# lancedb/lance

Measured on NVIDIA H100. Metric: ivf_pq_index_build_mvec_per_s, higher is better.
Workload: dtype f32

## Files before the change

### lance_b200/csrc/kmeans.cu

```cuda
#include <cooperative_groups.h>

#include <algorithm>
#include <cmath>
#include <limits>
#include <condition_variable>
#include <deque>
#include <functional>
#include <map>
#include <memory>
#include <mutex>
#include <queue>
#include <thread>
#include <unordered_map>

#include "../../include/lance_b200.h"

#include "assign.cuh"
#include "comm.cuh"
#include "common.cuh"
#include "exact.cuh"
#include "kmeans.cuh"
#include "tc_assign.cuh"
#include "tc_pq.cuh"

// ... 1051 lines not shown
  DevBuf<float> rn2;
  const bool pq_tc = small && ldx == B * ds && tc_pq_supported(n, ldx, B, ds, K, metric, x);
  TcPqPrepArgs pq_prep;
  bool pq_prepared = false;
  if (pq_tc) {
    rn2.alloc(n * B);
    tc_pq_residual_norms(x, nullptr, nullptr, n, B, nullptr, rn2.p);
    pq_prep = tc_pq_prep_args(B, ldx, &pqws);
  }
  sync_stream();
  const PollWords& words = PollWords::reset(B);
  auto iteration = [&]() {
    if (!small) {
      assign_f32_ex(x, n, ds, centroids, K, metric, bias.p, ids.p, dists.p, valid.p, nullptr, active_d.p, tcws);
    } else if (pq_tc) {
      tc_pq_assign(x, rn2.p, n, ldx, B, centroids, nullptr, nullptr, ids.p, dists.p, valid.p,
                   active_d.p, &pqws, pq_prepared);
      pq_prepared = true;
    } else {
      small_d_assign_f32(x, n, ldx, B, ds, centroids, K, metric, nullptr, nullptr, nullptr, nullptr,
                         ids.p, dists.p, valid.p, active_d.p);
    }
    ms.run(ids.p, valid.p, n, K, B, active_d.p);
    const int warp_update = (ds % 8 == 0 && ldx % 4 == 0 && (reinterpret_cast<uintptr_t>(x) & 15) == 0) ? 1 : 0;
    const unsigned ub = warp_update ? cdiv(BK * (uint64_t)(ds / 8), 4) : cdiv(BK * ds, 128);
    const unsigned sb = cdiv((uint64_t)BK * 32, 128);
    LB2_LAUNCH("kmeans_update_stats", update_stats_kernel, ub + sb, 128, 0, ub, x, ldx, ds, K, B, n,
               ms.members.p, ms.offsets.p, dist ? sums_p : centroids, dists.p, losses.p, radius.p,
               last_row.p, active_d.p, dist ? 0 : 1, warp_update, hints.p);
    if (dist) {
      LB2_LAUNCH("kmeans_pack_partials", pack_partials_kernel, cdiv(BK, 256), 256, 0, blob.p, xl, BK, ms.counts.p,
// ... 373 lines not shown
```

### lance_b200/csrc/tc_assign.cu

```cuda
#include <cuda_bf16.h>
#include <cuda_fp16.h>

#include "assign.cuh"
#include "common.cuh"
#include "exact.cuh"
#include "tc_assign.cuh"
#include "tc_common.cuh"

namespace lb2 {

namespace tc {

struct SmemLayout {
  uint32_t b_off, a_off, cnh_off, bar_off, total;
};
__host__ __device__ inline SmemLayout smem_layout(int nkc, int stages) {
  SmemLayout L;
  L.b_off = 0;
  L.a_off = nkc * B_CHUNK_BYTES;
  L.cnh_off = L.a_off + stages * A_STAGE_BYTES;
  L.bar_off = L.cnh_off + TN * 4;
  L.total = L.bar_off + (2 * MAX_STAGES + 1) * 8;
  return L;
}

__device__ __forceinline__ uint32_t verdict(float m1, float m2, float m3, float tau) {
  if (m1 - m2 > tau) return 0;
  if (m1 - m3 > tau) return 1;
  return 2;
}

__global__ void __launch_bounds__(NUM_THREADS, 1)
tc_filter_kernel(const __grid_constant__ CUtensorMap map_x, const __grid_constant__ CUtensorMap map_c,
                 uint64_t n, int nkc, int stages, const float* __restrict__ cnh_g,
                 const float* __restrict__ row_norm2, const float* __restrict__ cn2_g,
                 uint32_t* __restrict__ res, const uint8_t* __restrict__ active, float tau_scale) {
  if (active && !active[0]) return;
  extern __shared__ uint8_t smem_raw[];
  uint8_t* smem = smem_align1024(smem_raw);
  const SmemLayout L = smem_layout(nkc, stages);
  float* cnh = reinterpret_cast<float*>(smem + L.cnh_off);
  uint64_t* bars = reinterpret_cast<uint64_t*>(smem + L.bar_off);
  const uint32_t sb = smem_u32(smem);
  auto full_bar = [&](int s) { return smem_u32(&bars[s]); };
  auto empty_bar = [&](int s) { return smem_u32(&bars[MAX_STAGES + s]); };
  const uint32_t b_full = smem_u32(&bars[2 * MAX_STAGES]);

  const int warp = threadIdx.x >> 5, lane = threadIdx.x & 31;
  const uint64_t num_tiles = (n + TM - 1) / TM;

// ... 27 lines not shown
      for_units_producer(num_tiles, 1, [&](uint64_t tile, int) {
        for (int kc = 0; kc < nkc; ++kc) {
          mbar_wait_relaxed(empty_bar(s), ph ^ 1);
          mbar_expect_tx(full_bar(s), A_STAGE_BYTES);
          tma_load_2d(sb + L.a_off + s * A_STAGE_BYTES, &map_x, full_bar(s), kc * KC, (int)(tile * TM));
          if (++s == stages) { s = 0; ph ^= 1; }
        }
      });
    }
  } else {
    setmaxnreg_inc<CONSUMER_REGS>();
    const int w = (threadIdx.x >> 7) - 1;
    const float cmax2 = s_cmax2;
    float acc[128];
    mbar_wait(b_full, 0);
    for_units_consumer(num_tiles, 1, nkc, w, [&](uint64_t tile, int, uint64_t k, auto pass_turn) {
      mma_unit<0>(acc, nkc,
          [&](int kc, uint32_t& a_addr, uint32_t& b_addr) {
            const uint64_t kk = k + (uint64_t)kc;
            const int s = (int)(kk % (uint64_t)stages);
            mbar_wait(full_bar(s), (uint32_t)((kk / (uint64_t)stages) & 1));
            a_addr = sb + L.a_off + s * A_STAGE_BYTES;
            b_addr = sb + L.b_off + kc * B_CHUNK_BYTES;
            return s;
          },
          [&](int s) {
            __syncwarp();
            if (lane == 0) mbar_arrive(empty_bar(s));
          });
      pass_turn();
      float m[3];
      top3_frag(acc, cnh, m);
      if ((lane & 3) < 2) {
        const uint64_t row = tile * TM + frag_row(lane & 1);
        if (row < n) {
          const uint32_t flag = verdict(m[0], m[1], m[2], tau_scale * (row_norm2[row] + cmax2));
          res[row] = (__float_as_uint(m[0]) & 0xFFu) | ((__float_as_uint(m[1]) & 0xFFu) << 12) | (flag << 30);
        }
      }
    });
  }
}

constexpr int GEN_STAGES = 5;
constexpr int GEN_STAGE_BYTES = A_STAGE_BYTES + B_CHUNK_BYTES;

struct GenLayout {
  uint32_t stage_off, bar_off, total;
};
__host__ __device__ inline GenLayout gen_layout() {
  GenLayout L;
// ... 173 lines not shown
  for (int off = 16; off >= 1; off >>= 1) n2 += __shfl_xor_sync(0xffffffffu, n2, off);
  if (lane == 0) {
    cnh[k] = k < K ? -0.5f * (n2 + (bias ? bias[k] : 0.0f)) : -3.0e38f;
    cn2[k] = (k < K && n2 == n2) ? n2 : 0.0f;
  }
}

__global__ void row_norm_kernel(const float* __restrict__ x, uint64_t n, int d, float* __restrict__ out) {
  const uint64_t hw = ((uint64_t)blockIdx.x * blockDim.x + threadIdx.x) >> 4;
  const int l = threadIdx.x & 15;
  if (hw >= n) return;
  const float* v = x + hw * d;
  float s = 0.0f;
  for (int e = l * 4; e < d; e += 64) {
    const float4 f = *reinterpret_cast<const float4*>(v + e);
    s += f.x * f.x + f.y * f.y + f.z * f.z + f.w * f.w;
  }
  const unsigned mask = 0xffffu << (16 * ((threadIdx.x >> 4) & 1));
#pragma unroll
  for (int off = 8; off >= 1; off >>= 1) s += __shfl_xor_sync(mask, s, off, 16);
  if (l == 0) out[hw] = s;
}

__global__ void __launch_bounds__(256)
rerank_kernel(const float* __restrict__ x, uint64_t n, int d, const float* __restrict__ cent,
              const float* __restrict__ bias, const uint32_t* __restrict__ res,
              const uint32_t* __restrict__ res_hi, int need_dist,
              uint32_t* __restrict__ part, float* __restrict__ dist, uint8_t* __restrict__ valid,
              uint32_t* __restrict__ fb_rows, uint32_t* __restrict__ fb_count,
              const uint8_t* __restrict__ active, const uint32_t* __restrict__ src_list,
              const uint32_t* __restrict__ src_count, uint32_t src_cap, const float* __restrict__ val_in,
// ... 377 lines not shown
                   uint32_t* part, float* dist, uint8_t* valid, const uint8_t* active,
                   TcWorkspace& ws, const void* x16, int x16_dtype) {
  using namespace tc;
  const bool resident = tc_resident_shape(d, K);
  const int ntiles = (K + TN - 1) / TN, Kp = ntiles * TN;
  int stages = MAX_STAGES;
  size_t smem = gen_layout().total + 1024;
  if (resident) {
    SmemLayout L = smem_layout(d / KC, stages);
    while (stages > 2 && L.total + 1024 > ctx().smem_optin) L = smem_layout(d / KC, --stages);
    smem = L.total + 1024;
  }
  if (smem > ctx().smem_optin) fail(LB2_UNSUPPORTED, "tc_assign: shared memory");
  if (ws.cpad.n < (size_t)Kp * d) ws.cpad.alloc((size_t)Kp * d);
  if (ws.cnh.n < (size_t)2 * Kp + 1) ws.cnh.alloc((size_t)2 * Kp + 1);
  if (ws.row_norm2.n < n || ws.norm_src != x || ws.norm_n != n) {
    if (ws.row_norm2.n < n) ws.row_norm2.alloc(n);
    LB2_LAUNCH("tc_row_norms", row_norm_kernel, cdiv(n * 16, 256), 256, 0, x, n, d, ws.row_norm2.p);
    ws.norm_src = x;
    ws.norm_n = n;
  }
  const uint64_t res_n = resident ? n : 2 * n;
  if (ws.res.n < res_n) ws.res.alloc(res_n);
  if (ws.fb_rows.n < n) ws.fb_rows.alloc(n);
  if (ws.fb_count.n < 4) ws.fb_count.alloc(4);
  float* cnh = ws.cnh.p;
  float* cn2 = ws.cnh.p + Kp;
  float* cmax2 = ws.cnh.p + 2 * (size_t)Kp;
  if (resident) {
    const int Kp64 = (K + 63) / 64 * 64;
    if (ws.cT.n < (size_t)d * Kp64) ws.cT.alloc((size_t)d * Kp64);
    LB2_LAUNCH("tc_prep_centroids", prep_centroids_kernel, TN / 8, 256, 0, cent, K, d, bias, ws.cpad.p, cnh, cn2,
               ws.cT.p, Kp64, ws.fb_count.p);
// ... 16 lines not shown
  const unsigned grid = (unsigned)std::min<uint64_t>(tiles, (uint64_t)ctx().num_sms);
  const char* filter = resident ? "tc_filter" : opk ? "tc_filter_general16" : "tc_filter_general";
  if (opk) {
    if (ws.top1_val.n < n) ws.top1_val.alloc(n);
    const CUtensorMap map_x = make_map_2d_16(x16, opk == 2, n, d, TM);
    const CUtensorMap map_c = make_map_2d_16(ws.cpad16.p, opk == 2, Kp, d, TN);
    launch_general_dyn(opk, 0, grid, smem, map_x, map_c, n, d / (2 * KC), ntiles, cnh, ws.row_norm2.p, cmax2, ws.res.p,
                       ws.res.p + n, active, tau16_scale(d), nullptr, 0u, ws.top1_val.p, nullptr, nullptr, nullptr,
                       filter);
  } else {
    const CUtensorMap map_x = make_map_2d(x, n, d, TM);
    const CUtensorMap map_c = make_map_2d(ws.cpad.p, Kp, d, TN);
    if (resident) {
      set_smem(tc_filter_kernel, smem);
      LB2_LAUNCH(filter, tc_filter_kernel, grid, NUM_THREADS, smem, map_x, map_c, n, d / KC, stages, cnh,
                 ws.row_norm2.p, cn2, ws.res.p, active, TAU_TF32);
    } else {
      launch_general_dyn(0, 0, grid, smem, map_x, map_c, n, d / KC, ntiles, cnh, ws.row_norm2.p, cmax2, ws.res.p,
                         ws.res.p + n, active, TAU_TF32, nullptr, 0u, nullptr, nullptr, nullptr, nullptr, filter);
    }
  }
  LB2_LAUNCH("tc_rerank", rerank_kernel, cdiv(n * 16, 256), 256, 0, x, n, d, cent, bias, ws.res.p,
             (const uint32_t*)(resident ? nullptr : ws.res.p + n), dist != nullptr ? 1 : 0, part, dist, valid,
             ws.fb_rows.p, ws.fb_count.p, active, (const uint32_t*)nullptr, (const uint32_t*)nullptr, 0u,
             (const float*)nullptr, (float*)nullptr, (uint32_t*)nullptr, (uint32_t*)nullptr);
  const bool refined = tc_refine_and_fallback(x, n, d, cent, K, Kp, bias, ws.cpad.p, cnh, cmax2, part, dist, valid,
                                              active, ws, resident, opk, x16);
  if (getenv("LB2_TC_STATS") && *getenv("LB2_TC_STATS")) {
    std::vector<uint32_t> h(n);
    uint32_t c[3];
    d2h(h.data(), ws.res.p, n);
// ... 14 lines not shown
```

### lance_b200/csrc/tc_common.cuh

```cuda
#pragma once
#include <cuda.h>
#include <cudaTypedefs.h>
#include <stdint.h>
#include <stdio.h>

#include "common.cuh"

namespace lb2 {
namespace tc {

constexpr int TM = 64;
constexpr int TN = 256;
constexpr int KC = 32;
constexpr int A_STAGE_BYTES = TM * 128;
constexpr int B_CHUNK_BYTES = TN * 128;
constexpr int MAX_STAGES = 6;
constexpr int NUM_THREADS = 384;
constexpr int PRODUCER_REGS = 40, CONSUMER_REGS = 232;

__device__ __forceinline__ uint32_t smem_u32(const void* p) {
  return static_cast<uint32_t>(__cvta_generic_to_shared(p));
}
__device__ __forceinline__ void mbar_init(uint32_t bar, uint32_t count) {
  asm volatile("mbarrier.init.shared::cta.b64 [%0], %1;" ::"r"(bar), "r"(count));
// ... 86 lines not shown
      : "+f"(d[0]), "+f"(d[1]), "+f"(d[2]), "+f"(d[3]), "+f"(d[4]), "+f"(d[5]), "+f"(d[6]), "+f"(d[7]), "+f"(d[8]), "+f"(d[9]), "+f"(d[10]), "+f"(d[11]), "+f"(d[12]), "+f"(d[13]), "+f"(d[14]), "+f"(d[15]), "+f"(d[16]), "+f"(d[17]), "+f"(d[18]), "+f"(d[19]), "+f"(d[20]), "+f"(d[21]), "+f"(d[22]), "+f"(d[23]), "+f"(d[24]), "+f"(d[25]), "+f"(d[26]), "+f"(d[27]), "+f"(d[28]), "+f"(d[29]), "+f"(d[30]), "+f"(d[31]), "+f"(d[32]), "+f"(d[33]), "+f"(d[34]), "+f"(d[35]), "+f"(d[36]), "+f"(d[37]), "+f"(d[38]), "+f"(d[39]), "+f"(d[40]), "+f"(d[41]), "+f"(d[42]), "+f"(d[43]), "+f"(d[44]), "+f"(d[45]), "+f"(d[46]), "+f"(d[47]), "+f"(d[48]), "+f"(d[49]), "+f"(d[50]), "+f"(d[51]), "+f"(d[52]), "+f"(d[53]), "+f"(d[54]), "+f"(d[55]), "+f"(d[56]), "+f"(d[57]), "+f"(d[58]), "+f"(d[59]), "+f"(d[60]), "+f"(d[61]), "+f"(d[62]), "+f"(d[63])
      : "l"(a_desc), "l"(b_desc), "r"(scale_d));
}
__device__ __forceinline__ void wgmma_fence() { asm volatile("wgmma.fence.sync.aligned;" ::: "memory"); }
__device__ __forceinline__ void wgmma_commit() { asm volatile("wgmma.commit_group.sync.aligned;" ::: "memory"); }
template <int N>
__device__ __forceinline__ void wgmma_wait() { asm volatile("wgmma.wait_group.sync.aligned %0;" ::"n"(N) : "memory"); }
__device__ __forceinline__ void wgmma_wait_all() { wgmma_wait<0>(); }
template <int N = 128>
__device__ __forceinline__ void acc_fence(float* d) {
#pragma unroll
  for (int i = 0; i < N; ++i) asm volatile("" : "+f"(d[i])::"memory");
}
__device__ __forceinline__ uint8_t* smem_align1024(uint8_t* raw) {
  return raw + ((1024u - (smem_u32(raw) & 1023u)) & 1023u);
}
template <int OPK>
__device__ __forceinline__ void wgmma_op(float* d, uint64_t a_desc, uint64_t b_desc, uint32_t scale_d) {
  if (OPK == 0) wgmma_tf32(d, a_desc, b_desc, scale_d);
  else if (OPK == 1) wgmma_f16(d, a_desc, b_desc, scale_d);
  else wgmma_bf16(d, a_desc, b_desc, scale_d);
}
template <int OPK, class Stage, class Release>
__device__ __forceinline__ void mma_unit(float* d, int nkc, Stage&& stage, Release&& release) {
  acc_fence(d);
  int prev = -1;
  for (int kc = 0; kc < nkc; ++kc) {
    uint32_t a_addr, b_addr;
    const int s = stage(kc, a_addr, b_addr);
    __syncwarp();
// ... 182 lines not shown
```

### lance_b200/csrc/tc_pq.cu

```cuda
#include "assign.cuh"
#include "common.cuh"
#include "exact.cuh"
#include "tc_common.cuh"
#include "tc_pq.cuh"

namespace lb2 {
namespace tcpq {

using namespace tc;

constexpr int DS = 8;
constexpr int MAX_M_RESIDENT = 16;
constexpr int MAX_M = 256;
constexpr int CNH_CHUNK_BYTES = 4 * TN * 4;
constexpr int STREAM_STAGE_BYTES = A_STAGE_BYTES + B_CHUNK_BYTES + CNH_CHUNK_BYTES;

template <bool STREAM>
struct Pipe {
  static constexpr int CONSUMERS = STREAM ? 2 : 4;
  static constexpr int STAGES = STREAM ? 4 : 8;
  static constexpr int ACC_SETS = STREAM ? 2 : 1;
  static constexpr int THREADS = 128 * (1 + CONSUMERS);
  static constexpr int PRODUCER_REGS = STREAM ? 40 : 24;
  static constexpr int CONSUMER_REGS = STREAM ? 232 : 112;
  static_assert(STAGES % CONSUMERS == 0, "stages are dealt to the consumer warpgroups in turns");
  static_assert(128 * (PRODUCER_REGS + CONSUMERS * CONSUMER_REGS) <= THREADS * ((65536 / THREADS) & ~7),
                "register file");
};

struct Layout {
  uint32_t b_off, a_off, cnh_off, bar_off, cbm_off, misc_off, total;
  uint32_t stage_bytes;
};
__host__ __device__ inline Layout layout(int nkc, int M, bool stream) {
  Layout L;
  if (stream) {
    L.b_off = A_STAGE_BYTES;
    L.a_off = 0;
    L.cnh_off = A_STAGE_BYTES + B_CHUNK_BYTES;
    L.stage_bytes = STREAM_STAGE_BYTES;
    L.bar_off = Pipe<true>::STAGES * STREAM_STAGE_BYTES;
  } else {
    L.b_off = 0;
    L.a_off = nkc * B_CHUNK_BYTES;
    L.cnh_off = L.a_off + Pipe<false>::STAGES * A_STAGE_BYTES;
    L.stage_bytes = A_STAGE_BYTES;
    L.bar_off = L.cnh_off + M * TN * 4;
  }
  static_assert((2 * Pipe<false>::STAGES + 1) * 8 <= 256 && (2 * Pipe<true>::STAGES + 1) * 8 <= 256, "barriers");
  L.cbm_off = L.bar_off + 256;
  L.misc_off = L.cbm_off + MAX_M * 4;
  L.total = L.misc_off + MAX_M;
  return L;
}

__device__ __forceinline__ void bulk_load_1d(uint32_t dst, const void* src, uint32_t bytes, uint32_t bar) {
  asm volatile("cp.async.bulk.shared::cluster.global.mbarrier::complete_tx::bytes [%0], [%1], %2, [%3];"
               ::"r"(dst), "l"(src), "r"(bytes), "r"(bar)
               : "memory");
}

__device__ __forceinline__ const float4* swz(const uint8_t* tile, int r, int u) {
  return reinterpret_cast<const float4*>(tile + (r >> 3) * 1024 + (r & 7) * 128 + ((u ^ (r & 7)) << 4));
}

template <bool TRAIN, bool STREAM>
__global__ void __launch_bounds__(Pipe<STREAM>::THREADS, 1)
tc_pq_kernel(const __grid_constant__ CUtensorMap map_r, const __grid_constant__ CUtensorMap map_b,
             uint64_t n, int M, const float* __restrict__ cnh_g, const float* __restrict__ cbmax2,
             const float* __restrict__ rn2, const uint8_t* __restrict__ row_valid,
             uint8_t* __restrict__ codes, uint32_t* __restrict__ ids, float* __restrict__ dists,
             uint8_t* __restrict__ valid, uint32_t* __restrict__ fb_pairs,
             uint32_t* __restrict__ fb_count, const uint8_t* __restrict__ active) {
  using P = Pipe<STREAM>;
  constexpr int STAGES = P::STAGES;
  extern __shared__ uint8_t smem_raw[];
  uint8_t* smem = smem_align1024(smem_raw);
  const int nkc = M / 4;
  const Layout L = layout(nkc, M, STREAM);
  uint64_t* bars = reinterpret_cast<uint64_t*>(smem + L.bar_off);
  uint8_t* act_s = smem + L.misc_off;
  float* cbm_s = reinterpret_cast<float*>(smem + L.cbm_off);
  const uint32_t sb = smem_u32(smem);
  auto full_bar = [&](int s) { return smem_u32(&bars[s]); };
  auto empty_bar = [&](int s) { return smem_u32(&bars[STAGES + s]); };
  const uint32_t b_full = smem_u32(&bars[2 * STAGES]);

  const int warp = threadIdx.x >> 5, lane = threadIdx.x & 31;
  const uint64_t num_tiles = (n + TM - 1) / TM;

  if (!STREAM) {
    float* cnh = reinterpret_cast<float*>(smem + L.cnh_off);
    for (int i = threadIdx.x; i < M * TN; i += P::THREADS) cnh[i] = cnh_g[i];
  }
  int any_active = 0;
  for (int m = threadIdx.x; m < M; m += P::THREADS) {
    const uint8_t a = (!active || active[m]) ? 1 : 0;
    act_s[m] = a;
    cbm_s[m] = cbmax2[m];
    any_active |= a;
  }
  if (threadIdx.x == 32) {
    for (int s = 0; s < STAGES; ++s) {
      mbar_init(full_bar(s), 1);
      mbar_init(empty_bar(s), 4);
    }
    mbar_init(b_full, 1);
    asm volatile("fence.mbarrier_init.release.cluster;" ::: "memory");
  }
  any_active = __syncthreads_or(any_active);
  if (!any_active) return;
  auto chunk_mask = [&](int kc) -> uint32_t {
    const uint32_t w = reinterpret_cast<const uint32_t*>(act_s)[kc];
    return (w | (w >> 7) | (w >> 14) | (w >> 21)) & 0xFu;
  };

  if (warp < 4) {
    setmaxnreg_dec<P::PRODUCER_REGS>();
    if (threadIdx.x == 0) {
      if (!STREAM) {
// ... 3 lines not shown
      }
      int s = 0;
      uint32_t ph = 0;
      for (uint64_t item = blockIdx.x; item < num_tiles * nkc; item += gridDim.x) {
        const uint64_t tile = item / nkc;
        const int kc = (int)(item % nkc);
        if (chunk_mask(kc) == 0) continue;
        mbar_wait_relaxed(empty_bar(s), ph ^ 1);
        mbar_expect_tx(full_bar(s), STREAM ? STREAM_STAGE_BYTES : A_STAGE_BYTES);
        tma_load_2d(sb + L.a_off + s * L.stage_bytes, &map_r, full_bar(s), kc * KC, (int)(tile * TM));
        if (STREAM) {
          tma_load_2d(sb + L.b_off + s * L.stage_bytes, &map_b, full_bar(s), kc * KC, 0);
          bulk_load_1d(sb + L.cnh_off + s * L.stage_bytes, cnh_g + (size_t)kc * 4 * TN, CNH_CHUNK_BYTES,
                       full_bar(s));
        }
        if (++s == STAGES) { s = 0; ph ^= 1; }
      }
    }
  } else {
    setmaxnreg_inc<P::CONSUMER_REGS>();
    const uint32_t w = (threadIdx.x >> 7) - 1;
    if (!STREAM) mbar_wait(b_full, 0);
    const int h = lane & 1;
    const int rl = frag_row(h);
    float acc[P::ACC_SETS][64];
    uint32_t k = 0;
    for (uint64_t item = blockIdx.x; item < num_tiles * nkc; item += gridDim.x) {
      const uint64_t tile = item / nkc;
      const int kc = (int)(item % nkc);
      const uint32_t cm = chunk_mask(kc);
      if (cm == 0) continue;
      const bool mine = k % P::CONSUMERS == w;
      const int s = (int)(k % STAGES);
      const uint32_t ph = (k / STAGES) & 1;
      ++k;
      if (!mine) continue;
      const uint64_t row = tile * TM + rl;
      const bool decides = (lane & 3) < 2 && row < n;
      float4 rn4 = make_float4(0.0f, 0.0f, 0.0f, 0.0f);
      if (decides) rn4 = *reinterpret_cast<const float4*>(rn2 + row * M + 4 * kc);
      mbar_wait(full_bar(s), ph);
      const uint8_t* atile = smem + L.a_off + s * L.stage_bytes;
      const uint8_t* bt = smem + L.b_off + (STREAM ? s * L.stage_bytes : kc * B_CHUNK_BYTES);
      const float* cn4 = reinterpret_cast<const float*>(smem + L.cnh_off + (STREAM ? s * L.stage_bytes : kc * CNH_CHUNK_BYTES));
      const uint32_t a_addr = smem_u32(atile), b_addr = smem_u32(bt);
      auto decide = [&](int j, const float (&mm)[3]) {
        const int m = kc * 4 + j;
        if (decides) {
          const float m1 = mm[0], m2 = mm[1], m3 = mm[2];
          const float rn = j == 0 ? rn4.x : j == 1 ? rn4.y : j == 2 ? rn4.z : rn4.w;
          const float cbm = cbm_s[m];
          const float tau = 0.0029296875f * (rn + cbm);
          uint32_t flag = 2;
          if (m1 - m2 > tau) flag = 0;
          else if (m1 - m3 > tau) flag = 1;
          const uint32_t i1 = __float_as_uint(m1) & 0xFFu, i2 = __float_as_uint(m2) & 0xFFu;
// ... 101 lines not shown
  tc_pq_prep_block(cb + (size_t)m * TN * DS, m, a, s_n2);
}

__global__ void residual_norms_kernel(const float* x, const float* __restrict__ cent,
                                      const uint32_t* __restrict__ part, uint64_t n, int M,
                                      float* r_out, float* __restrict__ rn2) {
  const uint64_t g = (uint64_t)blockIdx.x * blockDim.x + threadIdx.x;
  if (g >= n * M) return;
  const uint64_t row = g / M;
  const int m = g % M;
  const int d = M * DS;
  const float4* xp = reinterpret_cast<const float4*>(x + row * d + m * DS);
  float4 a = xp[0], b = xp[1];
  if (cent) {
    const float4* cp = reinterpret_cast<const float4*>(cent + (size_t)part[row] * d + m * DS);
    const float4 ca = cp[0], cbv = cp[1];
    a.x = __fsub_rn(a.x, ca.x); a.y = __fsub_rn(a.y, ca.y); a.z = __fsub_rn(a.z, ca.z); a.w = __fsub_rn(a.w, ca.w);
    b.x = __fsub_rn(b.x, cbv.x); b.y = __fsub_rn(b.y, cbv.y); b.z = __fsub_rn(b.z, cbv.z); b.w = __fsub_rn(b.w, cbv.w);
  }
  if (r_out) {
    float4* rp = reinterpret_cast<float4*>(r_out + row * d + m * DS);
    rp[0] = a;
    rp[1] = b;
  }
  rn2[g] = a.x * a.x + a.y * a.y + a.z * a.z + a.w * a.w + b.x * b.x + b.y * b.y + b.z * b.z + b.w * b.w;
}

constexpr int FB_P = 2;
static __device__ __noinline__ void fb_exact_candidate(const float* rvq, const float* cp, int c, float& bv, uint32_t& bi) {
  float sacc = 0.0f;
#pragma unroll
  for (int t = 0; t < DS; ++t) sacc = f_add(sacc, sq_diff(rvq[t], cp[t]));
  const float v = f_add(sacc, 0.0f);
  if (v < bv) { bv = v; bi = (uint32_t)c; }
}
template <bool TRAIN>
__global__ void __launch_bounds__(256, 2)
pq_fallback_kernel(const float* __restrict__ r, uint64_t n, int M, const float* __restrict__ cb,
                   const uint32_t* __restrict__ pairs, const uint32_t* __restrict__ count,
                   const uint8_t* __restrict__ row_valid, uint8_t* __restrict__ codes,
                   uint32_t* __restrict__ ids, float* __restrict__ dists, uint8_t* __restrict__ valid) {
  __shared__ __align__(16) float cbs[TN * DS];
  __shared__ float cnh_s[TN];
  __shared__ float s_cmax;
  const int m = blockIdx.x;
  const uint32_t total = count[m];
  if (blockIdx.y * (16u * FB_P) >= total) return;
  {
    const float4* src = reinterpret_cast<const float4*>(cb + (size_t)m * TN * DS);
    float4* dst = reinterpret_cast<float4*>(cbs);
    for (int i = threadIdx.x; i < TN * DS / 4; i += 256) dst[i] = src[i];
  }
  __syncthreads();
// ... 10 lines not shown
    __syncthreads();
    if ((c & 31) == 0) atomicMax(reinterpret_cast<int*>(&s_cmax), __float_as_int(mx));
    __syncthreads();
  }
  const float cmax = s_cmax;
  const int l = threadIdx.x & 15;
  const unsigned mask = 0xffffu << (16 * ((threadIdx.x >> 4) & 1));
  const uint32_t* list = pairs + (size_t)m * n;
  for (uint32_t p0 = (blockIdx.y * 16u + (threadIdx.x >> 4)) * FB_P; p0 < total; p0 += gridDim.y * 16u * FB_P) {
    float rv[FB_P][DS], rn[FB_P];
    uint64_t rows[FB_P];
#pragma unroll
    for (int q = 0; q < FB_P; ++q) {
      rows[q] = list[min(p0 + q, total - 1)];
      const float* rp = r + rows[q] * (uint64_t)(M * DS) + m * DS;
      const float4 r0 = reinterpret_cast<const float4*>(rp)[0], r1 = reinterpret_cast<const float4*>(rp)[1];
      rv[q][0] = r0.x; rv[q][1] = r0.y; rv[q][2] = r0.z; rv[q][3] = r0.w;
      rv[q][4] = r1.x; rv[q][5] = r1.y; rv[q][6] = r1.z; rv[q][7] = r1.w;
      rn[q] = 0.0f;
#pragma unroll
      for (int t = 0; t < DS; ++t) rn[q] = fmaf(rv[q][t], rv[q][t], rn[q]);
    }
    float sc[FB_P][TN / 16], smax[FB_P];
#pragma unroll
    for (int q = 0; q < FB_P; ++q) smax[q] = __int_as_float(0xff800000);
#pragma unroll
    for (int i = 0; i < TN / 16; ++i) {
      const int c = l + 16 * i;
      const float4 c0 = reinterpret_cast<const float4*>(cbs + c * DS)[0];
      const float4 c1 = reinterpret_cast<const float4*>(cbs + c * DS)[1];
      const float cv[DS] = {c0.x, c0.y, c0.z, c0.w, c1.x, c1.y, c1.z, c1.w};
// ... 55 lines not shown
  if (ws->fb_count.n < (size_t)M) ws->fb_count.alloc(M);
  TcPqPrepArgs a;
  a.bm = ws->bm.p;
  a.cnh = ws->cnh.p;
  a.cbmax2 = ws->cnh.p + (size_t)M * tc::TN;
  a.fb_count = ws->fb_count.p;
  a.d = d;
  return a;
}
void tc_pq_prepare(const float* codebook, int M, int d, TcPqWorkspace* ws) {
  using namespace tcpq;
  const TcPqPrepArgs a = tc_pq_prep_args(M, d, ws);
  LB2_LAUNCH("tc_pq_prep_codebook", prep_codebook_kernel, M, tc::TN, 0, codebook, a);
}

void tc_pq_assign(const float* r, const float* rn2, uint64_t n, int d, int M, const float* codebook,
                  const uint8_t* row_valid, uint8_t* codes, uint32_t* ids, float* dists,
                  uint8_t* valid, const uint8_t* active, TcPqWorkspace* ws, bool prepared) {
  using namespace tcpq;
  const int nkc = M / 4;
  const bool stream = M > MAX_M_RESIDENT;
  const Layout L = layout(nkc, M, stream);
  const size_t smem = L.total + 1024;
  if (smem > ctx().smem_optin) fail(LB2_UNSUPPORTED, "tc_pq: shared memory");
  if (!prepared) tc_pq_prepare(codebook, M, d, ws);
  if (ws->fb_pairs.n < n * M) ws->fb_pairs.alloc(n * M);
  const CUtensorMap map_r = make_map_2d(r, n, d, tc::TM);
  const CUtensorMap map_b = make_map_2d(ws->bm.p, tc::TN, d, tc::TN);
  const uint64_t tiles = (n + tc::TM - 1) / tc::TM;
  const unsigned grid = (unsigned)std::min<uint64_t>(tiles * nkc, (uint64_t)ctx().num_sms);
  const float* cnh = ws->cnh.p;
  const float* cbmax2 = ws->cnh.p + (size_t)M * tc::TN;
  const dim3 fb_grid((unsigned)M, (unsigned)std::min<uint64_t>(cdiv(n, 16 * tcpq::FB_P), std::max(1, 8 * ctx().num_sms / M)));
#define LB2_PQ_FILTER(TRAINV, STREAMV)                                                                      \
  do {                                                                                                      \
    set_smem(tc_pq_kernel<TRAINV, STREAMV>, smem);                                                          \
    LB2_LAUNCH("tc_pq_filter", (tc_pq_kernel<TRAINV, STREAMV>), grid, Pipe<STREAMV>::THREADS, smem, map_r,   \
               map_b, n, M, cnh, cbmax2, rn2, row_valid, codes, ids, dists, valid, ws->fb_pairs.p,          \
               ws->fb_count.p, active);                                                                     \
  } while (0)
  if (codes) {
    if (stream) LB2_PQ_FILTER(false, true); else LB2_PQ_FILTER(false, false);
    LB2_LAUNCH("tc_pq_fallback", pq_fallback_kernel<false>, fb_grid, 256, 0, r, n, M, codebook,
               ws->fb_pairs.p, ws->fb_count.p, row_valid, codes, ids, dists, valid);
  } else {
    if (stream) LB2_PQ_FILTER(true, true); else LB2_PQ_FILTER(true, false);
    LB2_LAUNCH("tc_pq_fallback", pq_fallback_kernel<true>, fb_grid, 256, 0, r, n, M, codebook,
               ws->fb_pairs.p, ws->fb_count.p, row_valid, codes, ids, dists, valid);
  }
#undef LB2_PQ_FILTER
  if (getenv("LB2_TC_STATS") && *getenv("LB2_TC_STATS")) {
    std::vector<uint32_t> cm(M);
    d2h(cm.data(), ws->fb_count.p, M);
    sync_stream();
    uint64_t c = 0;
    for (int m = 0; m < M; ++m) c += cm[m];
    fprintf(stderr, "[lb2 tc_pq] n=%llu M=%d: exact-fallback pairs %.2f%%\n", (unsigned long long)n, M,
            100.0 * c / ((double)n * M));
  }
}

void pq_encode_dev(const float* x, uint64_t n, int d, int M, int ds, const float* codebook, int metric,
                   const float* cent, const uint32_t* part, const uint8_t* row_valid, uint8_t* codes) {
  if (n == 0) return;
  if (!tc_pq_supported(n, d, M, ds, 256, metric, x)) {
    small_d_assign_f32(x, n, d, M, ds, codebook, 256, metric, cent, part, row_valid, codes, nullptr,
                       nullptr, nullptr, nullptr);
    return;
  }
  TcPqWorkspace ws;
  const uint64_t chunk = std::max<uint64_t>(1ull << 16, (1ull << 28) / (uint64_t)d);
  DevBuf<float> r, rn2(std::min(n, chunk) * M);
  if (cent) r.alloc(std::min(n, chunk) * d);
  for (uint64_t r0 = 0; r0 < n; r0 += chunk) {
    const uint64_t rows = std::min(chunk, n - r0);
    const float* xs = x + r0 * d;
    tc_pq_residual_norms(xs, cent, part ? part + r0 : nullptr, rows, M, cent ? r.p : nullptr, rn2.p);
    tc_pq_assign(cent ? r.p : xs, rn2.p, rows, d, M, codebook, row_valid ? row_valid + r0 : nullptr,
                 codes + r0 * M, nullptr, nullptr, nullptr, nullptr, &ws);
  }
}

void tc_pq_residual_norms(const float* x, const float* cent, const uint32_t* part, uint64_t n, int M,
                          float* r_out, float* rn2) {
  LB2_LAUNCH("tc_pq_residual_norms", tcpq::residual_norms_kernel, cdiv(n * M, 256), 256, 0, x, cent,
             part, n, M, r_out, rn2);
}

}
```

### lance_b200/csrc/tc_pq.cuh

```cuda
#pragma once
#include <stdint.h>

#include "common.cuh"
namespace lb2 {
struct TcPqWorkspace {
  DevBuf<float> bm, cnh;
  DevBuf<uint32_t> fb_pairs, fb_count;
};
struct TcPqPrepArgs {
  float* bm = nullptr;
  float* cnh = nullptr;
  float* cbmax2 = nullptr;
  uint32_t* fb_count = nullptr;
  int d = 0;
};
#ifdef __CUDACC__
__device__ __forceinline__ void tc_pq_prep_block(const float* __restrict__ cb_m, int m, const TcPqPrepArgs& a,
                                                 float* s_n2 ) {
  const int c = threadIdx.x;
  const float* src = cb_m + (size_t)c * 8;
  float n2 = 0.0f;
#pragma unroll
  for (int t = 0; t < 8; ++t) {
    const float v = src[t];
// ... 3 lines not shown
  a.cnh[m * 256 + c] = -0.5f * n2;
  s_n2[c] = n2;
  __syncthreads();
  if (c < 32) {
    float mx = 0.0f;
    for (int i = c; i < 256; i += 32) mx = fmaxf(mx, s_n2[i]);
#pragma unroll
    for (int o = 16; o >= 1; o >>= 1) mx = fmaxf(mx, __shfl_xor_sync(0xffffffffu, mx, o));
    if (c == 0) a.cbmax2[m] = mx;
  }
}
#endif
bool tc_pq_supported(uint64_t n, int d, int M, int ds, int Kc, int metric, const float* x);
void tc_pq_residual_norms(const float* x, const float* cent, const uint32_t* part, uint64_t n, int M,
                          float* r_out, float* rn2);
void tc_pq_assign(const float* r, const float* rn2, uint64_t n, int d, int M, const float* codebook,
                  const uint8_t* row_valid, uint8_t* codes, uint32_t* ids, float* dists,
                  uint8_t* valid, const uint8_t* active, TcPqWorkspace* ws, bool prepared = false);
TcPqPrepArgs tc_pq_prep_args(int M, int d, TcPqWorkspace* ws);
void pq_encode_dev(const float* x, uint64_t n, int d, int M, int ds, const float* codebook, int metric,
                   const float* cent, const uint32_t* part, const uint8_t* row_valid, uint8_t* codes);
}
```

Measured before the change: 48.27.

## Fuse residual subtraction and row norms into TC PQ encode and filter kernels

In PQ encoding, the separate residual_norms pass, along with its residual buffer and rn2 buffer, is removed. Instead, the producer-side warps of the resident tc_pq kernel subtract the centroid in shared memory and compute sub-vector norms. A new ready barrier then gates the consumers. The fallback kernel recomputes residuals on the fly from cent and part. Separately, the IVF tc_filter_kernel computes row norms from the staged A tiles, so it no longer needs a dedicated row_norm kernel. These changes save global memory traffic and kernel launches, at the cost of extra shared-memory work in the producer and consumer paths and more complex synchronization.

Result: no change. 49.17 (median of 6 runs) (+1.9%).

```diff
diff --git a/lance_b200/csrc/kmeans.cu b/lance_b200/csrc/kmeans.cu
--- a/lance_b200/csrc/kmeans.cu
+++ b/lance_b200/csrc/kmeans.cu
@@ -1089,7 +1089,7 @@
     if (!small) {
       assign_f32_ex(x, n, ds, centroids, K, metric, bias.p, ids.p, dists.p, valid.p, nullptr, active_d.p, tcws);
     } else if (pq_tc) {
-      tc_pq_assign(x, rn2.p, n, ldx, B, centroids, nullptr, nullptr, ids.p, dists.p, valid.p,
+      tc_pq_assign(x, rn2.p, nullptr, nullptr, n, ldx, B, centroids, nullptr, nullptr, ids.p, dists.p, valid.p,
                    active_d.p, &pqws, pq_prepared);
       pq_prepared = true;
     } else {
diff --git a/lance_b200/csrc/tc_assign.cu b/lance_b200/csrc/tc_assign.cu
--- a/lance_b200/csrc/tc_assign.cu
+++ b/lance_b200/csrc/tc_assign.cu
@@ -30,10 +30,12 @@
   return 2;
 }
 
+__device__ __forceinline__ float sq4(float4 f) { return f.x * f.x + f.y * f.y + f.z * f.z + f.w * f.w; }
+
 __global__ void __launch_bounds__(NUM_THREADS, 1)
 tc_filter_kernel(const __grid_constant__ CUtensorMap map_x, const __grid_constant__ CUtensorMap map_c,
                  uint64_t n, int nkc, int stages, const float* __restrict__ cnh_g,
-                 const float* __restrict__ row_norm2, const float* __restrict__ cn2_g,
+                 const float* __restrict__ row_norm2, float* __restrict__ norm_out, const float* __restrict__ cn2_g,
                  uint32_t* __restrict__ res, const uint8_t* __restrict__ active, float tau_scale) {
   if (active && !active[0]) return;
   extern __shared__ uint8_t smem_raw[];
@@ -91,7 +93,10 @@
     const float cmax2 = s_cmax2;
     float acc[128];
     mbar_wait(b_full, 0);
+    const int nr = frag_row(lane & 1), nu = lane & 2 ? 4 : 0;
     for_units_consumer(num_tiles, 1, nkc, w, [&](uint64_t tile, int, uint64_t k, auto pass_turn) {
+      float np[2][4] = {{0.0f, 0.0f, 0.0f, 0.0f}, {0.0f, 0.0f, 0.0f, 0.0f}};
+      int kr = 0;
       mma_unit<0>(acc, nkc,
           [&](int kc, uint32_t& a_addr, uint32_t& b_addr) {
             const uint64_t kk = k + (uint64_t)kc;
@@ -102,16 +107,37 @@
             return s;
           },
           [&](int s) {
+            if (norm_out) {
+              const uint8_t* at = smem + L.a_off + s * A_STAGE_BYTES;
+#pragma unroll
+              for (int j = 0; j < 4; ++j) {
+                const float q = sq4(*swz(at, nr, nu + j));
+                if (kr & 1) np[1][j] += q;
+                else np[0][j] += q;
+              }
+              ++kr;
+            }
             __syncwarp();
             if (lane == 0) mbar_arrive(empty_bar(s));
           });
       pass_turn();
+      float rn_own = 0.0f;
+      if (norm_out) {
+        float a[4];
+#pragma unroll
+        for (int j = 0; j < 4; ++j) a[j] = np[0][j] + np[1][j];
+#pragma unroll
+        for (int j = 0; j < 4; ++j) a[j] += __shfl_xor_sync(0xffffffffu, a[j], 2);
+        rn_own = (a[0] + a[2]) + (a[1] + a[3]);
+      }
       float m[3];
       top3_frag(acc, cnh, m);
       if ((lane & 3) < 2) {
-        const uint64_t row = tile * TM + frag_row(lane & 1);
+        const uint64_t row = tile * TM + nr;
         if (row < n) {
-          const uint32_t flag = verdict(m[0], m[1], m[2], tau_scale * (row_norm2[row] + cmax2));
+          const float rn = norm_out ? rn_own : row_norm2[row];
+          if (norm_out) norm_out[row] = rn;
+          const uint32_t flag = verdict(m[0], m[1], m[2], tau_scale * (rn + cmax2));
           res[row] = (__float_as_uint(m[0]) & 0xFFu) | ((__float_as_uint(m[1]) & 0xFFu) << 12) | (flag << 30);
         }
       }
@@ -315,7 +341,7 @@
   float s = 0.0f;
   for (int e = l * 4; e < d; e += 64) {
     const float4 f = *reinterpret_cast<const float4*>(v + e);
-    s += f.x * f.x + f.y * f.y + f.z * f.z + f.w * f.w;
+    s += sq4(f);
   }
   const unsigned mask = 0xffffu << (16 * ((threadIdx.x >> 4) & 1));
 #pragma unroll
@@ -723,9 +749,11 @@
   if (smem > ctx().smem_optin) fail(LB2_UNSUPPORTED, "tc_assign: shared memory");
   if (ws.cpad.n < (size_t)Kp * d) ws.cpad.alloc((size_t)Kp * d);
   if (ws.cnh.n < (size_t)2 * Kp + 1) ws.cnh.alloc((size_t)2 * Kp + 1);
+  const bool filter_norms = resident && !active;
   if (ws.row_norm2.n < n || ws.norm_src != x || ws.norm_n != n) {
     if (ws.row_norm2.n < n) ws.row_norm2.alloc(n);
-    LB2_LAUNCH("tc_row_norms", row_norm_kernel, cdiv(n * 16, 256), 256, 0, x, n, d, ws.row_norm2.p);
+    if (!filter_norms)
+      LB2_LAUNCH("tc_row_norms", row_norm_kernel, cdiv(n * 16, 256), 256, 0, x, n, d, ws.row_norm2.p);
     ws.norm_src = x;
     ws.norm_n = n;
   }
@@ -772,7 +800,8 @@
     if (resident) {
       set_smem(tc_filter_kernel, smem);
       LB2_LAUNCH(filter, tc_filter_kernel, grid, NUM_THREADS, smem, map_x, map_c, n, d / KC, stages, cnh,
-                 ws.row_norm2.p, cn2, ws.res.p, active, TAU_TF32);
+                 filter_norms ? nullptr : ws.row_norm2.p, filter_norms ? ws.row_norm2.p : nullptr, cn2, ws.res.p,
+                 active, TAU_TF32);
     } else {
       launch_general_dyn(0, 0, grid, smem, map_x, map_c, n, d / KC, ntiles, cnh, ws.row_norm2.p, cmax2, ws.res.p,
                          ws.res.p + n, active, TAU_TF32, nullptr, 0u, nullptr, nullptr, nullptr, nullptr, filter);
diff --git a/lance_b200/csrc/tc_common.cuh b/lance_b200/csrc/tc_common.cuh
--- a/lance_b200/csrc/tc_common.cuh
+++ b/lance_b200/csrc/tc_common.cuh
@@ -124,6 +124,12 @@
 }
 __device__ __forceinline__ uint8_t* smem_align1024(uint8_t* raw) {
   return raw + ((1024u - (smem_u32(raw) & 1023u)) & 1023u);
+}
+__device__ __forceinline__ const float4* swz(const uint8_t* tile, int r, int u) {
+  return reinterpret_cast<const float4*>(tile + (r >> 3) * 1024 + (r & 7) * 128 + ((u ^ (r & 7)) << 4));
+}
+__device__ __forceinline__ float4* swz(uint8_t* tile, int r, int u) {
+  return const_cast<float4*>(swz(const_cast<const uint8_t*>(tile), r, u));
 }
 template <int OPK>
 __device__ __forceinline__ void wgmma_op(float* d, uint64_t a_desc, uint64_t b_desc, uint32_t scale_d) {
diff --git a/lance_b200/csrc/tc_pq.cu b/lance_b200/csrc/tc_pq.cu
--- a/lance_b200/csrc/tc_pq.cu
+++ b/lance_b200/csrc/tc_pq.cu
@@ -21,33 +21,35 @@
   static constexpr int STAGES = STREAM ? 4 : 8;
   static constexpr int ACC_SETS = STREAM ? 2 : 1;
   static constexpr int THREADS = 128 * (1 + CONSUMERS);
-  static constexpr int PRODUCER_REGS = STREAM ? 40 : 24;
+  static constexpr int PRODUCER_REGS = STREAM ? 40 : 32;
   static constexpr int CONSUMER_REGS = STREAM ? 232 : 112;
   static_assert(STAGES % CONSUMERS == 0, "stages are dealt to the consumer warpgroups in turns");
   static_assert(128 * (PRODUCER_REGS + CONSUMERS * CONSUMER_REGS) <= THREADS * ((65536 / THREADS) & ~7),
                 "register file");
 };
 
+constexpr int RN_STAGE_FLOATS = TM * 4;
 struct Layout {
-  uint32_t b_off, a_off, cnh_off, bar_off, cbm_off, misc_off, total;
+  uint32_t b_off, a_off, cnh_off, rn_off, bar_off, cbm_off, misc_off, total;
   uint32_t stage_bytes;
 };
-__host__ __device__ inline Layout layout(int nkc, int M, bool stream) {
+__host__ __device__ inline Layout layout(int nkc, int M, bool stream, bool fused) {
   Layout L;
   if (stream) {
     L.b_off = A_STAGE_BYTES;
     L.a_off = 0;
     L.cnh_off = A_STAGE_BYTES + B_CHUNK_BYTES;
     L.stage_bytes = STREAM_STAGE_BYTES;
-    L.bar_off = Pipe<true>::STAGES * STREAM_STAGE_BYTES;
+    L.rn_off = L.bar_off = Pipe<true>::STAGES * STREAM_STAGE_BYTES;
   } else {
     L.b_off = 0;
     L.a_off = nkc * B_CHUNK_BYTES;
     L.cnh_off = L.a_off + Pipe<false>::STAGES * A_STAGE_BYTES;
     L.stage_bytes = A_STAGE_BYTES;
-    L.bar_off = L.cnh_off + M * TN * 4;
-  }
-  static_assert((2 * Pipe<false>::STAGES + 1) * 8 <= 256 && (2 * Pipe<true>::STAGES + 1) * 8 <= 256, "barriers");
+    L.rn_off = L.cnh_off + M * TN * 4;
+    L.bar_off = L.rn_off + (fused ? Pipe<false>::STAGES * RN_STAGE_FLOATS * 4 : 0);
+  }
+  static_assert((3 * Pipe<false>::STAGES + 1) * 8 <= 256 && (2 * Pipe<true>::STAGES + 1) * 8 <= 256, "barriers");
   L.cbm_off = L.bar_off + 256;
   L.misc_off = L.cbm_off + MAX_M * 4;
   L.total = L.misc_off + MAX_M;
@@ -60,31 +62,38 @@
                : "memory");
 }
 
-__device__ __forceinline__ const float4* swz(const uint8_t* tile, int r, int u) {
-  return reinterpret_cast<const float4*>(tile + (r >> 3) * 1024 + (r & 7) * 128 + ((u ^ (r & 7)) << 4));
+__device__ __forceinline__ float4 sub4(float4 a, float4 c) {
+  return make_float4(__fsub_rn(a.x, c.x), __fsub_rn(a.y, c.y), __fsub_rn(a.z, c.z), __fsub_rn(a.w, c.w));
+}
+__device__ __forceinline__ float sub_norm2(float4 a, float4 b) {
+  return a.x * a.x + a.y * a.y + a.z * a.z + a.w * a.w + b.x * b.x + b.y * b.y + b.z * b.z + b.w * b.w;
 }
 
 template <bool TRAIN, bool STREAM>
 __global__ void __launch_bounds__(Pipe<STREAM>::THREADS, 1)
 tc_pq_kernel(const __grid_constant__ CUtensorMap map_r, const __grid_constant__ CUtensorMap map_b,
              uint64_t n, int M, const float* __restrict__ cnh_g, const float* __restrict__ cbmax2,
-             const float* __restrict__ rn2, const uint8_t* __restrict__ row_valid,
+             const float* __restrict__ rn2, const float* __restrict__ cent, const uint32_t* __restrict__ part,
+             const uint8_t* __restrict__ row_valid,
              uint8_t* __restrict__ codes, uint32_t* __restrict__ ids, float* __restrict__ dists,
              uint8_t* __restrict__ valid, uint32_t* __restrict__ fb_pairs,
              uint32_t* __restrict__ fb_count, const uint8_t* __restrict__ active) {
   using P = Pipe<STREAM>;
   constexpr int STAGES = P::STAGES;
+  constexpr bool FUSED = !TRAIN && !STREAM;
   extern __shared__ uint8_t smem_raw[];
   uint8_t* smem = smem_align1024(smem_raw);
   const int nkc = M / 4;
-  const Layout L = layout(nkc, M, STREAM);
+  const Layout L = layout(nkc, M, STREAM, FUSED);
   uint64_t* bars = reinterpret_cast<uint64_t*>(smem + L.bar_off);
   uint8_t* act_s = smem + L.misc_off;
   float* cbm_s = reinterpret_cast<float*>(smem + L.cbm_off);
+  float* rn_s = reinterpret_cast<float*>(smem + L.rn_off);
   const uint32_t sb = smem_u32(smem);
   auto full_bar = [&](int s) { return smem_u32(&bars[s]); };
   auto empty_bar = [&](int s) { return smem_u32(&bars[STAGES + s]); };
   const uint32_t b_full = smem_u32(&bars[2 * STAGES]);
+  auto ready_bar = [&](int s) { return smem_u32(&bars[2 * STAGES + 1 + s]); };
 
   const int warp = threadIdx.x >> 5, lane = threadIdx.x & 31;
   const uint64_t num_tiles = (n + TM - 1) / TM;
@@ -104,6 +113,7 @@
     for (int s = 0; s < STAGES; ++s) {
       mbar_init(full_bar(s), 1);
       mbar_init(empty_bar(s), 4);
+      if (FUSED) mbar_init(ready_bar(s), 96);
     }
     mbar_init(b_full, 1);
     asm volatile("fence.mbarrier_init.release.cluster;" ::: "memory");
@@ -137,6 +147,37 @@
           bulk_load_1d(sb + L.cnh_off + s * L.stage_bytes, cnh_g + (size_t)kc * 4 * TN, CNH_CHUNK_BYTES,
                        full_bar(s));
         }
+        if (++s == STAGES) { s = 0; ph ^= 1; }
+      }
+    } else if (FUSED && warp > 0) {
+      const int d = M * DS;
+      const uint32_t items = (uint32_t)num_tiles * nkc;
+      int s = 0;
+      uint32_t ph = 0;
+      for (uint32_t item = blockIdx.x; item < items; item += gridDim.x) {
+        const uint32_t tile = item / nkc;
+        const int kc = (int)(item % nkc);
+        if (chunk_mask(kc) == 0) continue;
+        mbar_wait_relaxed(full_bar(s), ph);
+        uint8_t* atile = smem + L.a_off + s * A_STAGE_BYTES;
+        for (int p = threadIdx.x - 32; p < RN_STAGE_FLOATS; p += 96) {
+          const int r = p >> 2, j = p & 3;
+          const uint32_t row = tile * TM + r;
+          if (row >= n) break;
+          float4* u0 = swz(atile, r, 2 * j);
+          float4* u1 = swz(atile, r, 2 * j + 1);
+          float4 a = *u0, b = *u1;
+          if (cent) {
+            const float4* c = reinterpret_cast<const float4*>(cent + (size_t)part[row] * d + kc * KC + j * DS);
+            a = sub4(a, c[0]);
+            b = sub4(b, c[1]);
+            *u0 = a;
+            *u1 = b;
+          }
+          rn_s[s * RN_STAGE_FLOATS + p] = sub_norm2(a, b);
+        }
+        asm volatile("fence.proxy.async.shared::cta;" ::: "memory");
+        mbar_arrive(ready_bar(s));
         if (++s == STAGES) { s = 0; ph ^= 1; }
       }
     }
@@ -161,8 +202,9 @@
       const uint64_t row = tile * TM + rl;
       const bool decides = (lane & 3) < 2 && row < n;
       float4 rn4 = make_float4(0.0f, 0.0f, 0.0f, 0.0f);
-      if (decides) rn4 = *reinterpret_cast<const float4*>(rn2 + row * M + 4 * kc);
-      mbar_wait(full_bar(s), ph);
+      if (!FUSED && decides) rn4 = *reinterpret_cast<const float4*>(rn2 + row * M + 4 * kc);
+      mbar_wait(FUSED ? ready_bar(s) : full_bar(s), ph);
+      if (FUSED && decides) rn4 = *reinterpret_cast<const float4*>(rn_s + s * RN_STAGE_FLOATS + rl * 4);
       const uint8_t* atile = smem + L.a_off + s * L.stage_bytes;
       const uint8_t* bt = smem + L.b_off + (STREAM ? s * L.stage_bytes : kc * B_CHUNK_BYTES);
       const float* cn4 = reinterpret_cast<const float*>(smem + L.cnh_off + (STREAM ? s * L.stage_bytes : kc * CNH_CHUNK_BYTES));
@@ -294,16 +336,15 @@
   float4 a = xp[0], b = xp[1];
   if (cent) {
     const float4* cp = reinterpret_cast<const float4*>(cent + (size_t)part[row] * d + m * DS);
-    const float4 ca = cp[0], cbv = cp[1];
-    a.x = __fsub_rn(a.x, ca.x); a.y = __fsub_rn(a.y, ca.y); a.z = __fsub_rn(a.z, ca.z); a.w = __fsub_rn(a.w, ca.w);
-    b.x = __fsub_rn(b.x, cbv.x); b.y = __fsub_rn(b.y, cbv.y); b.z = __fsub_rn(b.z, cbv.z); b.w = __fsub_rn(b.w, cbv.w);
+    a = sub4(a, cp[0]);
+    b = sub4(b, cp[1]);
   }
   if (r_out) {
     float4* rp = reinterpret_cast<float4*>(r_out + row * d + m * DS);
     rp[0] = a;
     rp[1] = b;
   }
-  rn2[g] = a.x * a.x + a.y * a.y + a.z * a.z + a.w * a.w + b.x * b.x + b.y * b.y + b.z * b.z + b.w * b.w;
+  rn2[g] = sub_norm2(a, b);
 }
 
 constexpr int FB_P = 2;
@@ -316,7 +357,8 @@
 }
 template <bool TRAIN>
 __global__ void __launch_bounds__(256, 2)
-pq_fallback_kernel(const float* __restrict__ r, uint64_t n, int M, const float* __restrict__ cb,
+pq_fallback_kernel(const float* __restrict__ r, const float* __restrict__ cent, const uint32_t* __restrict__ part,
+                   uint64_t n, int M, const float* __restrict__ cb,
                    const uint32_t* __restrict__ pairs, const uint32_t* __restrict__ count,
                    const uint8_t* __restrict__ row_valid, uint8_t* __restrict__ codes,
                    uint32_t* __restrict__ ids, float* __restrict__ dists, uint8_t* __restrict__ valid) {
@@ -357,7 +399,12 @@
     for (int q = 0; q < FB_P; ++q) {
       rows[q] = list[min(p0 + q, total - 1)];
       const float* rp = r + rows[q] * (uint64_t)(M * DS) + m * DS;
-      const float4 r0 = reinterpret_cast<const float4*>(rp)[0], r1 = reinterpret_cast<const float4*>(rp)[1];
+      float4 r0 = reinterpret_cast<const float4*>(rp)[0], r1 = reinterpret_cast<const float4*>(rp)[1];
+      if (cent) {
+        const float4* cp = reinterpret_cast<const float4*>(cent + (size_t)part[rows[q]] * (M * DS) + m * DS);
+        r0 = sub4(r0, cp[0]);
+        r1 = sub4(r1, cp[1]);
+      }
       rv[q][0] = r0.x; rv[q][1] = r0.y; rv[q][2] = r0.z; rv[q][3] = r0.w;
       rv[q][4] = r1.x; rv[q][5] = r1.y; rv[q][6] = r1.z; rv[q][7] = r1.w;
       rn[q] = 0.0f;
@@ -443,13 +490,14 @@
   LB2_LAUNCH("tc_pq_prep_codebook", prep_codebook_kernel, M, tc::TN, 0, codebook, a);
 }
 
-void tc_pq_assign(const float* r, const float* rn2, uint64_t n, int d, int M, const float* codebook,
-                  const uint8_t* row_valid, uint8_t* codes, uint32_t* ids, float* dists,
-                  uint8_t* valid, const uint8_t* active, TcPqWorkspace* ws, bool prepared) {
+void tc_pq_assign(const float* r, const float* rn2, const float* cent, const uint32_t* part, uint64_t n, int d,
+                  int M, const float* codebook, const uint8_t* row_valid, uint8_t* codes, uint32_t* ids,
+                  float* dists, uint8_t* valid, const uint8_t* active, TcPqWorkspace* ws, bool prepared) {
   using namespace tcpq;
   const int nkc = M / 4;
   const bool stream = M > MAX_M_RESIDENT;
-  const Layout L = layout(nkc, M, stream);
+  const bool fused = codes && !stream;
+  const Layout L = layout(nkc, M, stream, fused);
   const size_t smem = L.total + 1024;
   if (smem > ctx().smem_optin) fail(LB2_UNSUPPORTED, "tc_pq: shared memory");
   if (!prepared) tc_pq_prepare(codebook, M, d, ws);
@@ -465,16 +513,16 @@
   do {                                                                                                      \
     set_smem(tc_pq_kernel<TRAINV, STREAMV>, smem);                                                          \
     LB2_LAUNCH("tc_pq_filter", (tc_pq_kernel<TRAINV, STREAMV>), grid, Pipe<STREAMV>::THREADS, smem, map_r,   \
-               map_b, n, M, cnh, cbmax2, rn2, row_valid, codes, ids, dists, valid, ws->fb_pairs.p,          \
-               ws->fb_count.p, active);                                                                     \
+               map_b, n, M, cnh, cbmax2, rn2, cent, part, row_valid, codes, ids, dists, valid,              \
+               ws->fb_pairs.p, ws->fb_count.p, active);                                                     \
   } while (0)
   if (codes) {
     if (stream) LB2_PQ_FILTER(false, true); else LB2_PQ_FILTER(false, false);
-    LB2_LAUNCH("tc_pq_fallback", pq_fallback_kernel<false>, fb_grid, 256, 0, r, n, M, codebook,
+    LB2_LAUNCH("tc_pq_fallback", pq_fallback_kernel<false>, fb_grid, 256, 0, r, cent, part, n, M, codebook,
                ws->fb_pairs.p, ws->fb_count.p, row_valid, codes, ids, dists, valid);
   } else {
     if (stream) LB2_PQ_FILTER(true, true); else LB2_PQ_FILTER(true, false);
-    LB2_LAUNCH("tc_pq_fallback", pq_fallback_kernel<true>, fb_grid, 256, 0, r, n, M, codebook,
+    LB2_LAUNCH("tc_pq_fallback", pq_fallback_kernel<true>, fb_grid, 256, 0, r, cent, part, n, M, codebook,
                ws->fb_pairs.p, ws->fb_count.p, row_valid, codes, ids, dists, valid);
   }
 #undef LB2_PQ_FILTER
@@ -499,14 +547,23 @@
   }
   TcPqWorkspace ws;
   const uint64_t chunk = std::max<uint64_t>(1ull << 16, (1ull << 28) / (uint64_t)d);
-  DevBuf<float> r, rn2(std::min(n, chunk) * M);
-  if (cent) r.alloc(std::min(n, chunk) * d);
+  const bool fused = M <= tcpq::MAX_M_RESIDENT;
+  DevBuf<float> r, rn2;
+  if (!fused) rn2.alloc(std::min(n, chunk) * M);
+  if (!fused && cent) r.alloc(std::min(n, chunk) * d);
   for (uint64_t r0 = 0; r0 < n; r0 += chunk) {
     const uint64_t rows = std::min(chunk, n - r0);
     const float* xs = x + r0 * d;
-    tc_pq_residual_norms(xs, cent, part ? part + r0 : nullptr, rows, M, cent ? r.p : nullptr, rn2.p);
-    tc_pq_assign(cent ? r.p : xs, rn2.p, rows, d, M, codebook, row_valid ? row_valid + r0 : nullptr,
-                 codes + r0 * M, nullptr, nullptr, nullptr, nullptr, &ws);
+    const uint32_t* ps = part ? part + r0 : nullptr;
+    const uint8_t* vs = row_valid ? row_valid + r0 : nullptr;
+    if (fused) {
+      tc_pq_assign(xs, nullptr, cent, ps, rows, d, M, codebook, vs, codes + r0 * M, nullptr, nullptr, nullptr,
+                   nullptr, &ws);
+    } else {
+      tc_pq_residual_norms(xs, cent, ps, rows, M, cent ? r.p : nullptr, rn2.p);
+      tc_pq_assign(cent ? r.p : xs, rn2.p, nullptr, nullptr, rows, d, M, codebook, vs, codes + r0 * M, nullptr,
+                   nullptr, nullptr, nullptr, &ws);
+    }
   }
 }
 
diff --git a/lance_b200/csrc/tc_pq.cuh b/lance_b200/csrc/tc_pq.cuh
--- a/lance_b200/csrc/tc_pq.cuh
+++ b/lance_b200/csrc/tc_pq.cuh
@@ -41,9 +41,9 @@
 bool tc_pq_supported(uint64_t n, int d, int M, int ds, int Kc, int metric, const float* x);
 void tc_pq_residual_norms(const float* x, const float* cent, const uint32_t* part, uint64_t n, int M,
                           float* r_out, float* rn2);
-void tc_pq_assign(const float* r, const float* rn2, uint64_t n, int d, int M, const float* codebook,
-                  const uint8_t* row_valid, uint8_t* codes, uint32_t* ids, float* dists,
-                  uint8_t* valid, const uint8_t* active, TcPqWorkspace* ws, bool prepared = false);
+void tc_pq_assign(const float* r, const float* rn2, const float* cent, const uint32_t* part, uint64_t n, int d,
+                  int M, const float* codebook, const uint8_t* row_valid, uint8_t* codes, uint32_t* ids,
+                  float* dists, uint8_t* valid, const uint8_t* active, TcPqWorkspace* ws, bool prepared = false);
 TcPqPrepArgs tc_pq_prep_args(int M, int d, TcPqWorkspace* ws);
 void pq_encode_dev(const float* x, uint64_t n, int d, int M, int ds, const float* codebook, int metric,
                    const float* cent, const uint32_t* part, const uint8_t* row_valid, uint8_t* codes);
```
